# mburger-stsci/nexoclom

Measured on AMD Instinct MI355X. Metric: particle*steps/s, higher is better.
Workload: dtype f64

## Files before the change

### nexoclom_amd/csrc/nxc_api.hip

```cpp
#include <hip/hip_runtime.h>
#include <dlfcn.h>
#include <rccl/rccl.h>

#include <algorithm>
#include <atomic>
#include <cmath>
#include <cstddef>
#include <cstdio>
#include <cstdlib>
#include <cstring>
#include <ctime>
#include <limits>
#include <mutex>
#include <new>
#include <string>
#include <utility>
#include <vector>

#include "../../include/nexoclom_hip.h"
#include "nxc_camera_check.hpp"
#include "nxc_cube_check.hpp"
#include "nxc_desc_check.hpp"
#include "nxc_devbuf.hpp"
#include "nxc_image_block.hpp"
// ... 66 lines not shown
Rccl g_rccl;

int rccl_load()
{
    if (g_rccl.ok) return NXC_OK;
    const char *names[] = {"librccl.so.1", "librccl.so", "/opt/rocm/lib/librccl.so.1"};
    for (const char *nm : names) {
        g_rccl.lib = dlopen(nm, RTLD_NOW | RTLD_GLOBAL);
        if (g_rccl.lib) break;
    }
    if (!g_rccl.lib) return fail(NXC_ERR_RCCL, std::string("dlopen(librccl): ") + dlerror());
#define SYM(field, name)                                                                     \
    g_rccl.field = reinterpret_cast<decltype(g_rccl.field)>(dlsym(g_rccl.lib, name));        \
    if (!g_rccl.field) return fail(NXC_ERR_RCCL, std::string("dlsym ") + name + " failed");
    SYM(GetUniqueId, "ncclGetUniqueId")
    SYM(CommInitRank, "ncclCommInitRank")
    SYM(AllReduce, "ncclAllReduce")
    SYM(CommDestroy, "ncclCommDestroy")
    SYM(CommAbort, "ncclCommAbort")
    SYM(CommGetAsyncError, "ncclCommGetAsyncError")
    SYM(GetErrorString, "ncclGetErrorString")
#undef SYM
    g_rccl.ok = true;
    return NXC_OK;
}

#define NCCLCHK(expr)                                                                        \
    do {                                                                                     \
        ncclResult_t r_ = (expr);                                                            \
        if (r_ != ncclSuccess)                                                               \
            return fail(NXC_ERR_RCCL, std::string(#expr) + ": " + g_rccl.GetErrorString(r_)); \
    } while (0)

struct PackedLut {
    LutDesc desc{};
    std::vector<unsigned char> bytes;
};
struct LosLutCache {
    int64_t n = 0;
    std::vector<double> v, g;
    PackedLut lut;
};

int lut_cell_host(double x, double xbase, double inv_w, int ncell)
{
    const double s = (x - xbase) * inv_w;
    long long c;
    if (!(s >= 0.0)) c = 0;
    else if (s >= 2147483647.0) c = 2147483647ll;
    else c = (long long)s;
    return (int)std::min<long long>(c, ncell + 1);
}

unsigned long long ordered_key(double v)
{
    unsigned long long b;
    std::memcpy(&b, &v, sizeof b);
    return (b >> 63) ? ~b : (b | 0x8000000000000000ull);
}
double from_ordered_key(unsigned long long k)
{
    const unsigned long long b = (k >> 63) ? (k & 0x7fffffffffffffffull) : ~k;
    double v;
    std::memcpy(&v, &b, sizeof v);
    return v;
}

int pack_lut(const double *xp, const double *fp, int64_t n, PackedLut &out, const char *what,
             int cells_per_node = 4)
{
    if (n < 2 || n > 65000 || !xp || !fp)
        return fail(NXC_ERR_ARG, std::string(what) + ": table needs 2..65000 points");
    for (int64_t j = 0; j + 1 < n; j++)
        if (!(xp[j + 1] > xp[j]))
            return fail(NXC_ERR_ARG, std::string(what) + ": abscissae must be strictly ascending");
    for (int64_t j = 0; j < n; j++)
        if (!std::isfinite(xp[j]) || !std::isfinite(fp[j]))
            return fail(NXC_ERR_ARG, std::string(what) + ": table values must be finite");
    int ncell = 64;
    while (ncell < cells_per_node * n && ncell < 16384) ncell <<= 1;
    const int64_t rows = n + 2;
    const size_t cell_bytes = ((size_t)(ncell + 2) * sizeof(unsigned short) + 31) & ~size_t(31);
    out.bytes.assign((size_t)rows * 32 + cell_bytes, 0);
    double *rec = reinterpret_cast<double *>(out.bytes.data());
    double *fs = rec + 2 * rows;
    rec[0] = -std::numeric_limits<double>::max(); rec[1] = xp[0];
    fs[0] = fp[0]; fs[1] = 0.0;
    for (int64_t j = 0; j < n; j++) {
        const bool last = j + 1 == n;
        rec[2 * (j + 1)] = xp[j];
        rec[2 * (j + 1) + 1] = last ? HUGE_VAL : xp[j + 1];
        fs[2 * (j + 1)] = fp[j];
        fs[2 * (j + 1) + 1] = last ? 0.0 : (fp[j + 1] - fp[j]) / (xp[j + 1] - xp[j]);
        if (!std::isfinite(fs[2 * (j + 1) + 1]))
            return fail(NXC_ERR_ARG, std::string(what) + ": table slopes must be finite");
    }
    rec[2 * (n + 1)] = HUGE_VAL; rec[2 * (n + 1) + 1] = HUGE_VAL;
    fs[2 * (n + 1)] = fp[n - 1]; fs[2 * (n + 1) + 1] = 0.0;
    const double x0 = xp[0], xl = xp[n - 1];
    const double inv_w = (double)ncell / (xl - x0);
    const double xbase = x0 - (xl - x0) / (double)ncell;
    if (!std::isfinite(inv_w) || !std::isfinite(xbase) || !(xbase < x0))
        return fail(NXC_ERR_ARG, std::string(what) + ": abscissa range cannot be indexed");
    unsigned short *cell = reinterpret_cast<unsigned short *>(rec + 4 * rows);
    cell[0] = 0;
    const unsigned long long k_lo = ordered_key(-std::numeric_limits<double>::max());
    const unsigned long long k_hi = ordered_key(std::numeric_limits<double>::max());
    for (int c = 1; c <= ncell + 1; c++) {
        if (lut_cell_host(from_ordered_key(k_hi), xbase, inv_w, ncell) < c)
            return fail(NXC_ERR_ARG, std::string(what) + ": cell index is not onto");
        unsigned long long lo = k_lo, hi = k_hi;
        while (hi - lo > 1) {
            const unsigned long long mid = lo + (hi - lo) / 2;
            if (lut_cell_host(from_ordered_key(mid), xbase, inv_w, ncell) >= c) hi = mid;
            else lo = mid;
        }
        const double first = from_ordered_key(hi);
        const int64_t j = std::upper_bound(xp, xp + n, first) - xp;
        cell[c] = (unsigned short)j;
    }
    out.desc.rec = 0;
    out.desc.fs = 16 * (int)rows;
    out.desc.cell = 32 * (int)rows;
    out.desc.top = ncell + 1;
    out.desc.last = (int)n + 1;
    out.desc.xbase = xbase;
    out.desc.inv_w = inv_w;
    return NXC_OK;
}

int pack_lines(int n_lines, const double *const *v, const double *const *g, const int64_t *n, PackedLut *out)
{
    for (int l = 0; l < n_lines; l++) {
        int rc = pack_lut(v[l], g[l], n[l], out[l], "g-value table");
        if (rc) return rc;
    }
    return NXC_OK;
}

double sqrt_threshold(double e)
{
    if (!(e > 0) || !std::isfinite(e)) return e;
    double x = e * e;
    if (!std::isfinite(x)) return HUGE_VAL;
    while (std::sqrt(x) > e) x = std::nextafter(x, 0.0);
    while (std::sqrt(std::nextafter(x, HUGE_VAL)) <= e) x = std::nextafter(x, HUGE_VAL);
    return x;
}

StepW make_stepw(double h)
{
    StepW w{};
    w.h = h;
    for (int n = 0; n < 6; n++)
        for (int i = 0; i <= n; i++) w.w[n * (n + 1) / 2 + i] = h * Tableau::A[n + 1][i];
    return w;
}

void flush_all_pools();
struct HipAlloc {
    static inline thread_local hipError_t last = hipSuccess;
// ... 3787 lines not shown
```

### nexoclom_amd/csrc/nxc_device.hpp

```cpp
#pragma once
#include <hip/hip_runtime.h>
#include <stdint.h>
#include "nxc_math.hpp"
#include "nxc_fused_variant.hpp"

struct LutDesc {
    int rec, fs, cell;
    int top;
    int last;
    int pad_;
    double xbase;
    double inv_w;
};
typedef LutDesc LutView;

extern __shared__ __align__(32) unsigned char nxc_lds[];

#define NXC_LDS_AS __attribute__((address_space(3)))
#define NXC_GLOBAL_AS __attribute__((address_space(1)))
typedef double nxc_v2d __attribute__((ext_vector_type(2)));

NXC_DEV double lds_f64(int byte_off)
{
    return *(const NXC_LDS_AS double *)(unsigned)byte_off;
}
NXC_DEV int lds_u16(int byte_off)
{
    return *(const NXC_LDS_AS unsigned short *)(unsigned)byte_off;
}

NXC_DEV double2 lds_f64x2(int byte_off)
{
    const nxc_v2d v = *(const NXC_LDS_AS nxc_v2d *)(unsigned)byte_off;
    return make_double2(v.x, v.y);
}

NXC_DEV const LutView &lut_view(const LutDesc &d) { return d; }

NXC_DEV int lut_cell(const LutView &t, double x)
{
    const double s = (x - t.xbase) * t.inv_w;
    unsigned c;
    asm("v_cvt_u32_f64 %0, %1" : "=v"(c) : "v"(s));
    const unsigned top = (unsigned)t.top;
    return (int)(c > top ? top : c);
}

struct LutProbe {
    double x;
    int r;
    double2 a0, a1, b0, b1;
};

NXC_DEV void lut_probe_cell(const LutView &t, double x, LutProbe &p)
{
    p.x = x;
    p.r = lds_u16(t.cell + 2 * lut_cell(t, x));
}

NXC_DEV void lut_probe_rows(const LutView &t, LutProbe &p)
{
    const int ra = t.rec + 16 * p.r, rb = t.fs + 16 * p.r;
    p.a0 = lds_f64x2(ra); p.a1 = lds_f64x2(ra + 16);
    p.b0 = lds_f64x2(rb); p.b1 = lds_f64x2(rb + 16);
}

NXC_DEV LutProbe lut_probe(const LutView &t, double x)
{
    LutProbe p;
    lut_probe_cell(t, x, p);
    lut_probe_rows(t, p);
    return p;
}

NXC_DEV double lut_finish(const LutView &t, const LutProbe &p)
{
    const double x = p.x;
    const bool in0 = x < p.a0.y, in1 = x < p.a1.y;
    double xp = in0 ? p.a0.x : p.a1.x;
    double fp = in0 ? p.b0.x : p.b1.x;
    double sl = in0 ? p.b0.y : p.b1.y;
    if (__builtin_expect(!(in0 || in1), 0)) {
        int r = p.r + 1;
        while (r < t.last && x >= lds_f64(t.rec + 16 * r + 8)) ++r;
        const double2 aw = lds_f64x2(t.rec + 16 * r), bw = lds_f64x2(t.fs + 16 * r);
        xp = aw.x; fp = bw.x; sl = bw.y;
    }
    return sl * (x - xp) + fp;
}

NXC_DEV double lut_interp(const LutView &t, double x) { return lut_finish(t, lut_probe(t, x)); }

enum : int { LOSS_NONE = 0, LOSS_LIFETIME = 1, LOSS_PHOTO = 2 };

struct ForceK {
    double GM, vrplanet, photo, inv_lifetime;
    int grav, rad, loss, pad_;
    LutDesc tab;
};

NXC_DEV bool sunlit(double x, double y, double z)
{
    double s = x * x + z * z;
    return (s > 0x1.0000000000001p+0) || (y < 0.0);
}

template <bool FULL>
NXC_DEV void state_eval(const ForceK &F, const LutView &T, double x, double y, double z, double vy,
                        double &ax, double &ay, double &az, double &ion)
{
    const bool lit = sunlit(x, y, z);
    constexpr bool OVERLAP = FULL;
    LutProbe probe{};
    if (FULL || F.rad) lut_probe_cell(T, vy + F.vrplanet, probe);
    double gx = 0.0, gy = 0.0, gz = 0.0;
    if (FULL || F.grav) {
        const double s2 = (x * x + y * y) + z * z;
        const double nx = F.GM * x, ny = F.GM * y, nz = F.GM * z;
// ... 85 lines not shown
}

struct Tableau {
    static constexpr double A[7][7] = {
        {0, 0, 0, 0, 0, 0, 0},
        {0.2, 0, 0, 0, 0, 0, 0},
        {3. / 40., 9. / 40., 0, 0, 0, 0, 0},
        {44. / 45., -56. / 15., 32. / 9., 0, 0, 0, 0},
        {19372. / 6561., -25360. / 2187., 64448. / 6561., -212. / 729., 0, 0, 0},
        {9017. / 3168., -355. / 33., 46732. / 5247., 49. / 176., -5103. / 18656., 0, 0},
        {35. / 384., 0., 500. / 1113., 125. / 192., -2187. / 6784., 11. / 84., 0.}};
    static constexpr double B5[7] = {35. / 384., 0., 500. / 1113., 125. / 192., -2187. / 6784.,
                                     11. / 84., 0.};
    static constexpr double B4[7] = {5179. / 57600., 0., 7571. / 16695., 393. / 640.,
                                     -92097. / 339200., 187. / 2100., 1. / 40.};
};

struct StepW {
    double h;
    double w[21];
};

NXC_DEV double nxc_tab_fma(double w, double k, double acc)
{
#ifdef NXC_TABLEAU_TWO_ROUNDINGS
    return acc + w * k;
#else
    return __builtin_fma(w, k, acc);
#endif
}

template <bool DELTA, bool UNIFORM_H, bool FULL = false, bool NBODY = false>
NXC_DEV void rk5_step(const ForceK &F, const LutView &T, double (&s)[8], double h,
                      const StepW &W, double (&d)[8], const BodyK *Bd = nullptr,
                      const double *__restrict__ mp = nullptr)
{
    if (UNIFORM_H) h = W.h;
    double kv[6][3], ka[6][3], kl[6];
    const double x0 = s[1], y0 = s[2], z0 = s[3], vx0 = s[4], vy0 = s[5], vz0 = s[6];
    const double lf0 = nxc_log(s[7]);
    double px = x0, py = y0, pz = z0, vx = vx0, vy = vy0, vz = vz0, lf = lf0;
#pragma unroll
    for (int n = 0; n < 6; n++) {
        kv[n][0] = vx; kv[n][1] = vy; kv[n][2] = vz;
        state_eval<FULL>(F, T, px, py, pz, vy, ka[n][0], ka[n][1], ka[n][2], kl[n]);
        if (NBODY)
            bodies_eval(*Bd, mp, n, px, py, pz, vx, vy, vz, ka[n][0], ka[n][1], ka[n][2], kl[n]);
        double nx, ny, nz, nvx, nvy, nvz, nlf;
        {
            const double w = UNIFORM_H ? W.w[n * (n + 1) / 2] : h * Tableau::A[n + 1][0];
            nx = w * kv[0][0]; ny = w * kv[0][1]; nz = w * kv[0][2];
            nvx = w * ka[0][0]; nvy = w * ka[0][1]; nvz = w * ka[0][2];
            nlf = -(w * kl[0]);
        }
#pragma unroll
        for (int i = 1; i <= n; i++) {
            if (Tableau::A[n + 1][i] == 0.0) continue;
            const double w = UNIFORM_H ? W.w[n * (n + 1) / 2 + i] : h * Tableau::A[n + 1][i];
            nx = nxc_tab_fma(w, kv[i][0], nx);
            ny = nxc_tab_fma(w, kv[i][1], ny);
            nz = nxc_tab_fma(w, kv[i][2], nz);
            nvx = nxc_tab_fma(w, ka[i][0], nvx);
            nvy = nxc_tab_fma(w, ka[i][1], nvy);
            nvz = nxc_tab_fma(w, ka[i][2], nvz);
            nlf = nxc_tab_fma(-w, kl[i], nlf);
        }
        px = nx + x0; py = ny + y0; pz = nz + z0;
        vx = nvx + vx0; vy = nvy + vy0; vz = nvz + vz0;
        lf = nlf + lf0;
    }
    if (DELTA) {
        double e[7] = {0, 0, 0, 0, 0, 0, 0};
#pragma unroll
        for (int i = 0; i < 6; i++) {
            const double bd = Tableau::B5[i] - Tableau::B4[i];
            e[0] = nxc_tab_fma(bd, kv[i][0], e[0]);
            e[1] = nxc_tab_fma(bd, kv[i][1], e[1]);
            e[2] = nxc_tab_fma(bd, kv[i][2], e[2]);
            e[3] = nxc_tab_fma(bd, ka[i][0], e[3]);
            e[4] = nxc_tab_fma(bd, ka[i][1], e[4]);
            e[5] = nxc_tab_fma(bd, ka[i][2], e[5]);
            e[6] = nxc_tab_fma(bd, kl[i], e[6]);
        }
        d[0] = 0.0;
#pragma unroll
        for (int c = 0; c < 7; c++) d[c + 1] = __builtin_fabs(h * e[c]);
    }
    s[0] = (-h) + s[0];
    s[1] = px; s[2] = py; s[3] = pz; s[4] = vx; s[5] = vy; s[6] = vz;
    s[7] = nxc_exp(lf);
}
// ... 305 lines not shown
    R.vrplanet = G.vrplanet;
    R.xedges = (int)G.xedges_off; R.zedges = (int)G.zedges_off;
    R.nx = G.nx; R.nz = G.nz;
    R.x_lo = lds_f64(R.xedges); R.x_hi = lds_f64(R.xedges + 8 * R.nx);
    R.z_lo = lds_f64(R.zedges); R.z_hi = lds_f64(R.zedges + 8 * R.nz);
    R.x_inv_step = G.x_inv_step; R.z_inv_step = G.z_inv_step;
    R.quantity = G.quantity; R.n_lines = G.n_lines; R.downcast = G.downcast_f32;
    R.x_is_x = wave_uniform(G.x_is_x);
#ifdef NXC_EXPERIMENT_KNOBS
    R.dbg = G.dbg;
#else
    R.dbg = 0;
#endif
    R.vrplanet = wave_uniform(R.vrplanet);
    R.x_lo = wave_uniform(R.x_lo); R.x_hi = wave_uniform(R.x_hi);
    R.z_lo = wave_uniform(R.z_lo); R.z_hi = wave_uniform(R.z_hi);
    R.x_inv_step = wave_uniform(R.x_inv_step); R.z_inv_step = wave_uniform(R.z_inv_step);
    R.xedges = wave_uniform(R.xedges); R.zedges = wave_uniform(R.zedges);
    R.nx = wave_uniform(R.nx); R.nz = wave_uniform(R.nz);
    R.quantity = wave_uniform(R.quantity); R.n_lines = wave_uniform(R.n_lines);
    R.downcast = wave_uniform(R.downcast);
#ifdef NXC_EXPERIMENT_KNOBS
    R.dbg = wave_uniform(R.dbg);
#endif
    return R;
}

NXC_DEV double nxc_div_const(double n, double d, double y)
{
    if (!((nxc_mid_range(n) || n == 0.0) && y == y)) return n / d;
    return nxc_div_seeded(n, d, y);
}

NXC_DEV int bin_index(double v, int edges, int n, double lo, double hi, double inv_step)
{
    if (!(v >= lo) || !(v <= hi)) return -1;
    int k = (int)((v - lo) * inv_step);
    k = k > n - 1 ? n - 1 : k;
    const double e0 = lds_f64(edges + 8 * k), e1 = lds_f64(edges + 8 * k + 8);
    if (__builtin_expect(!((v >= e0) && (v < e1)), 0)) {
        while (k > 0 && v < lds_f64(edges + 8 * k)) --k;
        while (k < n - 1 && v >= lds_f64(edges + 8 * (k + 1))) ++k;
    }
    return k;
}

NXC_DEV double f32_round_trip(double v) { return (double)(float)v; }

NXC_DEV int half_swap(int v, bool upper)
{
    const auto r = __builtin_amdgcn_permlane32_swap(v, v, false, false);
    return upper ? (int)r[0] : (int)r[1];
}

NXC_DEV void image_add_pairs(bool has, int pix, double w, double *__restrict__ acc2)
{
    if (__ballot(has) == 0) return;
    const bool upper = (threadIdx.x & 32) != 0;
    const int ppix = half_swap(has ? pix : -1, upper);
    const bool own = has && w != 0.0;
    const bool partner = ppix >= 0;
    {
        const bool act = upper ? partner : own;
        if (act)
            unsafeAtomicAdd(&acc2[2ll * (upper ? ppix : pix) + (upper ? 1 : 0)], upper ? 1.0 : w);
    }
    {
        const bool act = upper ? own : partner;
        if (act)
            unsafeAtomicAdd(&acc2[2ll * (upper ? pix : ppix) + (upper ? 0 : 1)], upper ? w : 1.0);
    }
}

NXC_DEV double half_swap_f64(double v, bool upper)
{
    return __hiloint2double(half_swap(__double2hiint(v), upper), half_swap(__double2loint(v), upper));
}

NXC_DEV void add_record_pairs(bool has, int rec, double a, double b, double *__restrict__ rec2)
{
    if (__ballot(has) == 0) return;
    const bool upper = (threadIdx.x & 32) != 0;
    const int prec = half_swap(has ? rec : -1, upper);
    const double pb = half_swap_f64(b, upper);
    const bool partner = prec >= 0;
    {
        const bool act = upper ? partner : has;
        if (act)
            unsafeAtomicAdd(&rec2[2ll * (upper ? prec : rec) + (upper ? 1 : 0)], upper ? pb : a);
    }
    {
        const bool act = upper ? has : partner;
        if (act)
            unsafeAtomicAdd(&rec2[2ll * (upper ? rec : prec) + (upper ? 0 : 1)], upper ? a : pb);
    }
}

NXC_DEV bool image_locate_core_xz(const ImageK &G, const ImageRegs &R, double x, double y, double z,
                                  double vy, double frac, double &radvel_out, double &fw_out,
                                  unsigned long long &nonfinite, int &ix_out, int &iz_out)
{
    const double radvel = vy + R.vrplanet;
    double xo, yo, zo;
    if (R.x_is_x) {
        xo = x;
        yo = G.M[4] * y + G.M[5] * z;
        zo = G.M[7] * y + G.M[8] * z;
    } else {
        xo = (G.M[0] * x + G.M[1] * y) + G.M[2] * z;
        yo = (G.M[3] * x + G.M[4] * y) + G.M[5] * z;
        zo = (G.M[6] * x + G.M[7] * y) + G.M[8] * z;
    }
    const int ix = bin_index(xo, R.xedges, R.nx, R.x_lo, R.x_hi, R.x_inv_step);
    const int iz = bin_index(zo, R.zedges, R.nz, R.z_lo, R.z_hi, R.z_inv_step);
    if (ix < 0 || iz < 0) {
        if (!(__builtin_fabs(frac) <= 1.7976931348623157e308) || radvel != radvel) nonfinite++;
        return false;
    }
    const double s_obs = xo * xo + zo * zo;
    const bool inview = (s_obs > 0x1.0000000000001p+0) || (yo < 0.0);
    frac = inview ? frac : frac * 0.0;
    if (R.quantity != 0)
        frac = sunlit(x, y, z) ? frac : frac * 0.0;
    radvel_out = radvel;
    fw_out = frac;
    ix_out = ix; iz_out = iz;
    return true;
}

NXC_DEV int image_locate_core(const ImageK &G, const ImageRegs &R, double x, double y, double z,
                              double vy, double frac, double &radvel_out, double &fw_out,
                              unsigned long long &nonfinite)
{
    int ix = 0, iz = 0;
    if (!image_locate_core_xz(G, R, x, y, z, vy, frac, radvel_out, fw_out, nonfinite, ix, iz))
        return -1;
    return ix * R.nz + iz;
}

NXC_DEV int image_locate(const ImageK &G, const ImageRegs &R, double x, double y, double z,
                         double vy, double frac, double &radvel_out, double &fw_out,
                         unsigned long long &nonfinite)
{
    if (R.downcast) {
        x = f32_round_trip(x); y = f32_round_trip(y); z = f32_round_trip(z);
        vy = f32_round_trip(vy); frac = f32_round_trip(frac);
    }
    return image_locate_core(G, R, x, y, z, vy, frac, radvel_out, fw_out, nonfinite);
}

NXC_DEV bool image_frame_test(const ImageK &G, const ImageRegs &R, double x, double y, double z,
                              double vy, double frac, float &xf, float &yf, float &zf,
                              unsigned long long &nonfinite)
{
    xf = (float)x; yf = (float)y; zf = (float)z;
    const double xd = xf, yd = yf, zd = zf;
    double xo, zo;
    if (R.x_is_x) {
        xo = xd;
        zo = G.M[7] * yd + G.M[8] * zd;
    } else {
        xo = (G.M[0] * xd + G.M[1] * yd) + G.M[2] * zd;
        zo = (G.M[6] * xd + G.M[7] * yd) + G.M[8] * zd;
    }
    const bool inside = (xo >= R.x_lo) && (xo <= R.x_hi) && (zo >= R.z_lo) && (zo <= R.z_hi);
    if (!inside && (!(__builtin_fabs(frac) < 0x1.ffffffp127) || vy != vy)) nonfinite++;
    return inside;
}
// ... 235 lines not shown
```

### nexoclom_amd/csrc/nxc_image_block.hpp

```cpp
#pragma once
#include <cstddef>
#include <cstdint>
#include <vector>

#include "../../include/nexoclom_hip.h"

template <class Lut>
Lut placed_lut(Lut d, size_t base)
{
    d.rec += (int)base; d.fs += (int)base; d.cell += (int)base;
    return d;
}

template <class Lut>
struct ImageBlock {
    int n_lines = 0;
    Lut line[NXC_MAX_LINES]{};
    size_t xedges = 0, zedges = 0, bytes = 0;
};

template <class Image, class Packed>
auto append_image_block(std::vector<unsigned char> &out, Image &G, int64_t nx, int64_t nz,
                        const double *xedges, const double *zedges, int n_lines, const Packed *luts)
    -> ImageBlock<decltype(luts->desc)>
{
    ImageBlock<decltype(luts->desc)> b;
    const size_t start = out.size();
    b.n_lines = n_lines;
    for (int l = 0; l < n_lines; l++) {
        b.line[l] = placed_lut(luts[l].desc, out.size() - start);
        out.insert(out.end(), luts[l].bytes.begin(), luts[l].bytes.end());
    }
    b.xedges = out.size() - start;
    const unsigned char *xe = reinterpret_cast<const unsigned char *>(xedges);
    out.insert(out.end(), xe, xe + (nx + 1) * sizeof(double));
    b.zedges = out.size() - start;
    const unsigned char *ze = reinterpret_cast<const unsigned char *>(zedges);
    out.insert(out.end(), ze, ze + (nz + 1) * sizeof(double));
    b.bytes = out.size() - start;
    G.nx = (int)nx;
    G.nz = (int)nz;
    G.n_lines = n_lines;
    G.x_lo = xedges[0];
// ... 14 lines not shown
```

### nexoclom_amd/csrc/nxc_kernels.hpp

```cpp
#pragma once
#include "nxc_device.hpp"
#include "nxc_fused_variant.hpp"
#include "nxc_source_limits.hpp"
#include "nxc_tile_plan.hpp"

struct DevCounters {
    unsigned long long particle_steps, samples, samples_binned, nonfinite, bad_step, neg_frac,
        unfinished, queue_head;
    unsigned long long wave_trips;
#ifdef NXC_STAMPS
    unsigned long long stamp[8];
#endif
};

#ifdef NXC_STAMPS
NXC_DEV unsigned long long nxc_stamp()
{
    unsigned long long t;
    __builtin_amdgcn_sched_barrier(0);
    asm volatile("s_memtime %0\n\ts_waitcnt lgkmcnt(0)" : "=s"(t) : : "memory");
    __builtin_amdgcn_sched_barrier(0);
    return t;
}
#define NXC_STAMP(k) do { const unsigned long long t_ = nxc_stamp(); seg[k] += t_ - t_prev; t_prev = t_; } while (0)
// ... 91 lines not shown
    int hi = __builtin_amdgcn_readfirstlane((int)(v >> 32));
    return ((long long)hi << 32) | (unsigned int)lo;
}

__global__ void __launch_bounds__(NXC_BLOCK)
k_state(ForceK F, const unsigned char *__restrict__ blob, int64_t stage_bytes, int64_t n,
        const double *__restrict__ x, const double *__restrict__ y, const double *__restrict__ z,
        const double *__restrict__ vy, double *__restrict__ ax, double *__restrict__ ay,
        double *__restrict__ az, double *__restrict__ ion)
{
    stage_tables(blob, stage_bytes);
    const LutView T = lut_view(F.tab);
    for (int64_t i = (int64_t)blockIdx.x * blockDim.x + threadIdx.x; i < n;
         i += (int64_t)gridDim.x * blockDim.x) {
        double a0, a1, a2, l;
        state_eval<false>(F, T, x[i], y[i], z[i], vy[i], a0, a1, a2, l);
        ax[i] = a0; ay[i] = a1; az[i] = a2; ion[i] = l;
    }
}

template <bool DELTA>
__global__ void __launch_bounds__(NXC_BLOCK)
k_rk5_step(ForceK F, const unsigned char *__restrict__ blob, int64_t stage_bytes, int64_t n,
           const double *__restrict__ in, const double *__restrict__ hstep,
           double *__restrict__ out, double *__restrict__ delta)
{
    stage_tables(blob, stage_bytes);
    const LutView T = lut_view(F.tab);
    for (int64_t i = (int64_t)blockIdx.x * blockDim.x + threadIdx.x; i < n;
         i += (int64_t)gridDim.x * blockDim.x) {
        double s[8], d[8];
#pragma unroll
        for (int c = 0; c < 8; c++) s[c] = in[c * n + i];
        rk5_step<DELTA, false>(F, T, s, hstep[i], StepW{}, d);
#pragma unroll
        for (int c = 0; c < 8; c++) out[c * n + i] = s[c];
        if (DELTA) {
#pragma unroll
            for (int c = 0; c < 8; c++) delta[c * n + i] = d[c];
        }
    }
}

constexpr int NXC_REC_DOUBLES = 10;
constexpr int NXC_REC_FLOATS = 10;
typedef float nxc_v4f __attribute__((ext_vector_type(4)));
typedef float nxc_v2f __attribute__((ext_vector_type(2)));
typedef float nxc_v4f_a8 __attribute__((ext_vector_type(4), aligned(8)));

template <int ROWS>
NXC_DEV void store_record(void *__restrict__ rec, long long row, const double (&s)[8],
                          double lossfrac, long long id)
{
    if (ROWS == 2) {
        float *p = static_cast<float *>(rec) + row * NXC_REC_FLOATS;
        nxc_v4f a, b;
        nxc_v2f c;
        a.x = (float)s[0]; a.y = (float)s[1]; a.z = (float)s[2]; a.w = (float)s[3];
        b.x = (float)s[4]; b.y = (float)s[5]; b.z = (float)s[6]; b.w = (float)s[7];
        c.x = (float)lossfrac; c.y = __int_as_float((int)id);
        *reinterpret_cast<nxc_v4f_a8 *>(p) = a;
        *reinterpret_cast<nxc_v4f_a8 *>(p + 4) = b;
        *reinterpret_cast<nxc_v2f *>(p + 8) = c;
    } else {
        nxc_v2d *p = reinterpret_cast<nxc_v2d *>(static_cast<double *>(rec) + row * NXC_REC_DOUBLES);
        nxc_v2d a, b, c, d, e;
        a.x = s[0]; a.y = s[1]; b.x = s[2]; b.y = s[3]; c.x = s[4]; c.y = s[5]; d.x = s[6]; d.y = s[7];
// ... 146 lines not shown
                        stage[10 * NXC_CHUNK + lane] = __longlong_as_double(o1 - o0);
                    }
                }
                if (lane == 0) pending = claim(L.head);
                __builtin_amdgcn_fence(__ATOMIC_ACQUIRE, "wavefront");
                __builtin_amdgcn_wave_barrier();
            }
            const int room = c_cnt - c_pos;
            const int take = room < (want - served) ? room : want - served;
            if (need && rank >= served && rank < served + take) {
                const int slot = c_pos + (rank - served);
                mine = __double_as_longlong(stage[8 * NXC_CHUNK + slot]);
#pragma unroll
                for (int c = 0; c < 8; c++) s[c] = stage[c * NXC_CHUNK + slot];
                if (ROWS) {
                    *row0 = __double_as_longlong(stage[9 * NXC_CHUNK + slot]);
                    *nrow = __double_as_longlong(stage[10 * NXC_CHUNK + slot]);
                }
            }
            c_pos += take;
            served += take;
        }
        return mine;
    }
};

template <int IMAGE>
NXC_DEV bool image_pop(ImageQueue &queue, int imgq_off, const ImageRegs &IR, int &p, double &rv,
                       double &fw, unsigned long long &nonfinite)
{
    if (IMAGE == 2) {
        double x = 0, y = 0, z = 0, vy = 0, frac = 0;
        const bool ok = queue.pop_sample(imgq_off, x, y, z, vy, frac);
        if (ok) p = image_locate_core(lds_header().G, IR, x, y, z, vy, frac, rv, fw, nonfinite);
        return ok && p >= 0;
    }
    return queue.pop(imgq_off, p, rv, fw);
}

template <int IMAGE, bool BOUNCE, bool FULL, bool NBODY = false, int ROWS = 0, bool STREAMED = false>
__global__ void __launch_bounds__(NXC_BLOCK_PERSIST)
k_const_fused(ForceK F, const unsigned char *__restrict__ blob,
              int64_t stage_bytes, int64_t n, const double *__restrict__ soa0,
              const unsigned *__restrict__ order, int64_t first_id, int64_t n_iter,
              double edge2, double *__restrict__ final_out,
              long long *__restrict__ steps_out, double *__restrict__ acc2,
              DevCounters *__restrict__ ctr, const double *__restrict__ moon_pos = nullptr,
              const long long *__restrict__ offsets = nullptr, void *__restrict__ rec = nullptr,
              const unsigned long long *__restrict__ avail = nullptr)
{
    static_assert(!(IMAGE && ROWS), "the rows pass has no image");
    static_assert(!(STREAMED && (ROWS || BOUNCE || NBODY)), "the streamed pass is the plain one");
    stage_tables_and_args(blob, stage_bytes, soa0, order, final_out, steps_out, &ctr->queue_head, n,
                          offsets, STREAMED ? avail : nullptr);
    const LutView T = lut_view(F.tab);
    ImageRegs IR{};
    if (IMAGE) IR = image_regs(lds_header().G);
    ImageQueue queue;
    unsigned my_steps = 0, my_samples = 0, my_binned = 0;
    unsigned long long my_nonfinite = 0;
    WaveQueue q;
    q.start();
    const bool want_out = __builtin_amdgcn_readfirstlane(
        (final_out != nullptr || steps_out != nullptr) ? 1 : 0) != 0;
    const int wave_off = (int)((stage_bytes + 31) & ~31ll) +
                         (threadIdx.x >> 6) * (ROWS ? NXC_WAVE_LDS_BYTES_ROWS : NXC_WAVE_LDS_BYTES);
    const int stage_off = wave_off, imgq_off = wave_off + NXC_WAVE_STAGE_BYTES;
    bool has = false, fresh = false;
    long long id = -1, row0 = 0, nrow = 0;
    double lossfrac = 0.0;
    unsigned my_overrun = 0, my_trips = 0;
    int k = 0, nbounce = 0;
    const int n_it = n_iter > 0x7fffffffll ? 0x7fffffff : (int)n_iter;
    double s[8], d[8];
#ifdef NXC_STAMPS
    unsigned long long seg[8] = {0, 0, 0, 0, 0, 0, 0, 0}, t_prev = nxc_stamp();
#endif
    for (;;) {
#ifdef NXC_REFILL_MIN
        const unsigned long long free_ = __ballot(!has);
        const bool serve = __popcll(free_) >= NXC_REFILL_MIN || free_ == ~0ull;
        const long long got = serve ? q.refill<ROWS != 0, STREAMED>(!has, stage_off, s, &row0, &nrow) : -1;
#else
        const long long got = q.refill<ROWS != 0, STREAMED>(!has, stage_off, s, &row0, &nrow);
#endif
        if (got >= 0) { id = got; k = 0; has = true; fresh = true; nbounce = 0; lossfrac = 0.0; }
        if (__ballot(has) == 0) break;
        my_trips++;
        NXC_STAMP(0);
        int p = -1;
        double rv = 0.0, fw = 0.0;
        bool inframe = false;
        float qx = 0.f, qy = 0.f, qz = 0.f;
        if (has) {
            const double before = s[7];
            if (!fresh) {
                if (NBODY) {
                    const BodyK *Bd = &lds_header().Bd;
                    const double *mp = moon_pos + (long long)k * (2 * Bd->n_moons);
                    rk5_step<false, true, FULL, true>(F, T, s, 0.0, lds_header().W, d, Bd, mp);
                    apply_fate<false, true>(s, edge2, 0ull, nbounce, my_nonfinite, Bd, mp);
                } else {
                    rk5_step<false, true, FULL>(F, T, s, 0.0, lds_header().W, d);
                    apply_fate<BOUNCE>(s, edge2, (unsigned long long)(first_id + id), nbounce, my_nonfinite);
                }
#ifdef NXC_PROBE_VMOV
                {
                    int junk;
#pragma unroll
                    for (int j = 0; j < NXC_PROBE_VMOV; j++) asm volatile("v_mov_b32 %0, 0x12345" : "=v"(junk));
                }
#endif
#ifdef NXC_PROBE_FMA
                {
                    double j0 = s[1], j1 = s[2], j2 = s[3], j3 = s[4];
#pragma unroll
                    for (int j = 0; j < NXC_PROBE_FMA / 4; j++) {
                        asm volatile("v_fma_f64 %0, %0, %0, %0" : "+v"(j0));
                        asm volatile("v_fma_f64 %0, %0, %0, %0" : "+v"(j1));
                        asm volatile("v_fma_f64 %0, %0, %0, %0" : "+v"(j2));
                        asm volatile("v_fma_f64 %0, %0, %0, %0" : "+v"(j3));
                    }
                }
#endif
                k++; my_steps++;
                if (ROWS) lossfrac = (lossfrac + before) - s[7];
            }
            NXC_STAMP(1);
            fresh = false;
            const bool live = s[7] > 0.0;
            if (ROWS && live) {
                if (k < nrow) store_record<ROWS>(rec, row0 + k, s, lossfrac, id);
                else my_overrun++;
            }
            if (IMAGE && live) {
                my_samples++;
// ... 228 lines not shown
        if (__ballot(has) == 0) {
            if (!FAIR || !keeper || settled) break;
            const int simd = hw_simd();
            bool open = false;
            if (lane < nw) {
                const unsigned c = M.ld(M.hdr(lane));
                open = c == NXC_VAR_PENDING || (c != 0u && M.hdr(lane)[1] == (unsigned)simd && M.hdr(lane)[2] == 0u);
            }
            if (__ballot(open) == 0) break;
            __builtin_amdgcn_s_sleep(8);
            continue;
        }
        my_trips++;
        if (FAIR && !settled && (my_trips & 3u) == 0) {
            const unsigned long long t = __builtin_amdgcn_s_memrealtime();
            const int pr = (int)(((t >> NXC_VAR_PRIO_SHIFT) + (unsigned long long)hw_slot()) % 3ull);
            if (pr != prio) {
                prio = pr;
                if (pr == 2) __builtin_amdgcn_s_setprio(2);
                else if (pr == 1) __builtin_amdgcn_s_setprio(1);
                else __builtin_amdgcn_s_setprio(0);
            }
        }
        if (has) {
            bool done = !(s[0] > resolution && s[7] > 0.0);
            if (!done && it >= max_steps) { my_unfinished++; done = true; }
            if (!done) {
                const double h = __builtin_fmin(s[0], hs);
                if (!(h > 0.0)) { my_bad++; done = true; }
                else {
                    double t[8], d[8];
#pragma unroll
                    for (int c = 0; c < 8; c++) t[c] = s[c];
                    rk5_step<true, false, FULL>(F, T, t, h, StepW{}, d);
                    my_steps++; it++;
                    const double fscale = resf + __builtin_fabs(t[7]) * resf;
                    double e = d[0];
                    bool finite = true;
#pragma unroll
                    for (int c = 1; c <= 7; c++) {
                        const double scale = c <= 3 ? resx + __builtin_fabs(t[c]) * resx
                                           : c <= 6 ? resv + __builtin_fabs(t[c]) * resv : fscale;
                        const double q = nxc_div(d[c], scale);
                        finite = finite && (__builtin_fabs(q) <= 1.7976931348623157e308);
                        e = __builtin_fmax(e, q);
                    }
                    if (!finite) e = __builtin_nan("");
                    if (!(__builtin_fabs(e) <= 1.7976931348623157e308)) { my_nonfinite++; done = true; }
                    else {
                        if (t[7] < 0.0 && e < 1.0) my_neg++;
                        if ((t[7] - s[7] > fscale) && (e > 1.0)) e = 1.1;
                        double hold = h;
                        if (e < 1e-7) { e = 1.0; hold = h * 10; }
                        if (e < 1.0) {
                            { int nb_ = 0; apply_fate<false>(t, outeredge, 0ull, nb_, my_nonfinite); }
#pragma unroll
                            for (int c = 0; c < 8; c++) s[c] = t[c];
                        } else {
                            const double hn = 0.95 * hold * nxc_pow_m025(e);
                            if (!(__builtin_fabs(hn) <= 1.7976931348623157e308)) { my_bad++; done = true; }
                            else hs = __builtin_fmax(hn, 0.1 * hold);
                        }
                    }
                }
            }
            if (done) {
#pragma unroll
// ... 2046 lines not shown
```

Before: 33.84 billion.

## Fold LUT cell index into FMA and read RK weights from LDS

Precomputes c0 = -xbase*inv_w so the LUT cell lookup becomes a single FMA, and stores the fs-row offset relative to rec so the descriptor keeps one fewer base register. The RK5 step now loads its uniform weights and h straight from LDS at an offset instead of taking a StepW struct by value, with asm barriers to steer register and scalar/vector placement. Image binning in the in-frame sample path drops its redundant range checks through a template flag. Together these aim to cut VGPR pressure and ALU work per step, at the cost of extra LDS loads and small rounding differences in cell boundaries, which the host-side packer is updated to match.

```diff
diff --git a/nexoclom_amd/csrc/nxc_api.hip b/nexoclom_amd/csrc/nxc_api.hip
--- a/nexoclom_amd/csrc/nxc_api.hip
+++ b/nexoclom_amd/csrc/nxc_api.hip
@@ -122,101 +122,17 @@
             return fail(NXC_ERR_RCCL, std::string(#expr) + ": " + g_rccl.GetErrorString(r_)); \
     } while (0)
 
-struct PackedLut {
-    LutDesc desc{};
-    std::vector<unsigned char> bytes;
-};
 struct LosLutCache {
     int64_t n = 0;
     std::vector<double> v, g;
     PackedLut lut;
 };
 
-int lut_cell_host(double x, double xbase, double inv_w, int ncell)
-{
-    const double s = (x - xbase) * inv_w;
-    long long c;
-    if (!(s >= 0.0)) c = 0;
-    else if (s >= 2147483647.0) c = 2147483647ll;
-    else c = (long long)s;
-    return (int)std::min<long long>(c, ncell + 1);
-}
-
-unsigned long long ordered_key(double v)
-{
-    unsigned long long b;
-    std::memcpy(&b, &v, sizeof b);
-    return (b >> 63) ? ~b : (b | 0x8000000000000000ull);
-}
-double from_ordered_key(unsigned long long k)
-{
-    const unsigned long long b = (k >> 63) ? (k & 0x7fffffffffffffffull) : ~k;
-    double v;
-    std::memcpy(&v, &b, sizeof v);
-    return v;
-}
-
 int pack_lut(const double *xp, const double *fp, int64_t n, PackedLut &out, const char *what,
              int cells_per_node = 4)
 {
-    if (n < 2 || n > 65000 || !xp || !fp)
-        return fail(NXC_ERR_ARG, std::string(what) + ": table needs 2..65000 points");
-    for (int64_t j = 0; j + 1 < n; j++)
-        if (!(xp[j + 1] > xp[j]))
-            return fail(NXC_ERR_ARG, std::string(what) + ": abscissae must be strictly ascending");
-    for (int64_t j = 0; j < n; j++)
-        if (!std::isfinite(xp[j]) || !std::isfinite(fp[j]))
-            return fail(NXC_ERR_ARG, std::string(what) + ": table values must be finite");
-    int ncell = 64;
-    while (ncell < cells_per_node * n && ncell < 16384) ncell <<= 1;
-    const int64_t rows = n + 2;
-    const size_t cell_bytes = ((size_t)(ncell + 2) * sizeof(unsigned short) + 31) & ~size_t(31);
-    out.bytes.assign((size_t)rows * 32 + cell_bytes, 0);
-    double *rec = reinterpret_cast<double *>(out.bytes.data());
-    double *fs = rec + 2 * rows;
-    rec[0] = -std::numeric_limits<double>::max(); rec[1] = xp[0];
-    fs[0] = fp[0]; fs[1] = 0.0;
-    for (int64_t j = 0; j < n; j++) {
-        const bool last = j + 1 == n;
-        rec[2 * (j + 1)] = xp[j];
-        rec[2 * (j + 1) + 1] = last ? HUGE_VAL : xp[j + 1];
-        fs[2 * (j + 1)] = fp[j];
-        fs[2 * (j + 1) + 1] = last ? 0.0 : (fp[j + 1] - fp[j]) / (xp[j + 1] - xp[j]);
-        if (!std::isfinite(fs[2 * (j + 1) + 1]))
-            return fail(NXC_ERR_ARG, std::string(what) + ": table slopes must be finite");
-    }
-    rec[2 * (n + 1)] = HUGE_VAL; rec[2 * (n + 1) + 1] = HUGE_VAL;
-    fs[2 * (n + 1)] = fp[n - 1]; fs[2 * (n + 1) + 1] = 0.0;
-    const double x0 = xp[0], xl = xp[n - 1];
-    const double inv_w = (double)ncell / (xl - x0);
-    const double xbase = x0 - (xl - x0) / (double)ncell;
-    if (!std::isfinite(inv_w) || !std::isfinite(xbase) || !(xbase < x0))
-        return fail(NXC_ERR_ARG, std::string(what) + ": abscissa range cannot be indexed");
-    unsigned short *cell = reinterpret_cast<unsigned short *>(rec + 4 * rows);
-    cell[0] = 0;
-    const unsigned long long k_lo = ordered_key(-std::numeric_limits<double>::max());
-    const unsigned long long k_hi = ordered_key(std::numeric_limits<double>::max());
-    for (int c = 1; c <= ncell + 1; c++) {
-        if (lut_cell_host(from_ordered_key(k_hi), xbase, inv_w, ncell) < c)
-            return fail(NXC_ERR_ARG, std::string(what) + ": cell index is not onto");
-        unsigned long long lo = k_lo, hi = k_hi;
-        while (hi - lo > 1) {
-            const unsigned long long mid = lo + (hi - lo) / 2;
-            if (lut_cell_host(from_ordered_key(mid), xbase, inv_w, ncell) >= c) hi = mid;
-            else lo = mid;
-        }
-        const double first = from_ordered_key(hi);
-        const int64_t j = std::upper_bound(xp, xp + n, first) - xp;
-        cell[c] = (unsigned short)j;
-    }
-    out.desc.rec = 0;
-    out.desc.fs = 16 * (int)rows;
-    out.desc.cell = 32 * (int)rows;
-    out.desc.top = ncell + 1;
-    out.desc.last = (int)n + 1;
-    out.desc.xbase = xbase;
-    out.desc.inv_w = inv_w;
-    return NXC_OK;
+    const std::string why = pack_lut_rows(xp, fp, n, out, what, cells_per_node);
+    return why.empty() ? NXC_OK : fail(NXC_ERR_ARG, why);
 }
 
 int pack_lines(int n_lines, const double *const *v, const double *const *g, const int64_t *n, PackedLut *out)
diff --git a/nexoclom_amd/csrc/nxc_device.hpp b/nexoclom_amd/csrc/nxc_device.hpp
--- a/nexoclom_amd/csrc/nxc_device.hpp
+++ b/nexoclom_amd/csrc/nxc_device.hpp
@@ -3,15 +3,8 @@
 #include <stdint.h>
 #include "nxc_math.hpp"
 #include "nxc_fused_variant.hpp"
-
-struct LutDesc {
-    int rec, fs, cell;
-    int top;
-    int last;
-    int pad_;
-    double xbase;
-    double inv_w;
-};
+#include "nxc_lut_pack.hpp"
+
 typedef LutDesc LutView;
 
 extern __shared__ __align__(32) unsigned char nxc_lds[];
@@ -39,7 +32,7 @@
 
 NXC_DEV int lut_cell(const LutView &t, double x)
 {
-    const double s = (x - t.xbase) * t.inv_w;
+    const double s = __builtin_fma(x, t.inv_w, t.c0);
     unsigned c;
     asm("v_cvt_u32_f64 %0, %1" : "=v"(c) : "v"(s));
     const unsigned top = (unsigned)t.top;
@@ -60,7 +53,7 @@
 
 NXC_DEV void lut_probe_rows(const LutView &t, LutProbe &p)
 {
-    const int ra = t.rec + 16 * p.r, rb = t.fs + 16 * p.r;
+    const int ra = t.rec + 16 * p.r, rb = ra + t.to_fs;
     p.a0 = lds_f64x2(ra); p.a1 = lds_f64x2(ra + 16);
     p.b0 = lds_f64x2(rb); p.b1 = lds_f64x2(rb + 16);
 }
@@ -82,8 +75,9 @@
     double sl = in0 ? p.b0.y : p.b1.y;
     if (__builtin_expect(!(in0 || in1), 0)) {
         int r = p.r + 1;
+        asm volatile("" : "+v"(r));
         while (r < t.last && x >= lds_f64(t.rec + 16 * r + 8)) ++r;
-        const double2 aw = lds_f64x2(t.rec + 16 * r), bw = lds_f64x2(t.fs + 16 * r);
+        const double2 aw = lds_f64x2(t.rec + 16 * r), bw = lds_f64x2(t.rec + 16 * r + t.to_fs);
         xp = aw.x; fp = bw.x; sl = bw.y;
     }
     return sl * (x - xp) + fp;
@@ -235,10 +229,15 @@
 
 template <bool DELTA, bool UNIFORM_H, bool FULL = false, bool NBODY = false>
 NXC_DEV void rk5_step(const ForceK &F, const LutView &T, double (&s)[8], double h,
-                      const StepW &W, double (&d)[8], const BodyK *Bd = nullptr,
+                      int w_at, double (&d)[8], const BodyK *Bd = nullptr,
                       const double *__restrict__ mp = nullptr)
 {
-    if (UNIFORM_H) h = W.h;
+    int zero = 0;
+    if (UNIFORM_H) asm volatile("" : "+v"(zero));
+    const int w0 = zero + w_at + (int)offsetof(StepW, w);
+    if (UNIFORM_H) h = lds_f64(zero + w_at + (int)offsetof(StepW, h));
+    LutView Tv = T;
+    if (FULL) asm volatile("" : "+v"(Tv.c0));
     double kv[6][3], ka[6][3], kl[6];
     const double x0 = s[1], y0 = s[2], z0 = s[3], vx0 = s[4], vy0 = s[5], vz0 = s[6];
     const double lf0 = nxc_log(s[7]);
@@ -246,12 +245,12 @@
 #pragma unroll
     for (int n = 0; n < 6; n++) {
         kv[n][0] = vx; kv[n][1] = vy; kv[n][2] = vz;
-        state_eval<FULL>(F, T, px, py, pz, vy, ka[n][0], ka[n][1], ka[n][2], kl[n]);
+        state_eval<FULL>(F, Tv, px, py, pz, vy, ka[n][0], ka[n][1], ka[n][2], kl[n]);
         if (NBODY)
             bodies_eval(*Bd, mp, n, px, py, pz, vx, vy, vz, ka[n][0], ka[n][1], ka[n][2], kl[n]);
         double nx, ny, nz, nvx, nvy, nvz, nlf;
         {
-            const double w = UNIFORM_H ? W.w[n * (n + 1) / 2] : h * Tableau::A[n + 1][0];
+            const double w = UNIFORM_H ? lds_f64(w0 + 8 * (n * (n + 1) / 2)) : h * Tableau::A[n + 1][0];
             nx = w * kv[0][0]; ny = w * kv[0][1]; nz = w * kv[0][2];
             nvx = w * ka[0][0]; nvy = w * ka[0][1]; nvz = w * ka[0][2];
             nlf = -(w * kl[0]);
@@ -259,7 +258,7 @@
 #pragma unroll
         for (int i = 1; i <= n; i++) {
             if (Tableau::A[n + 1][i] == 0.0) continue;
-            const double w = UNIFORM_H ? W.w[n * (n + 1) / 2 + i] : h * Tableau::A[n + 1][i];
+            const double w = UNIFORM_H ? lds_f64(w0 + 8 * (n * (n + 1) / 2 + i)) : h * Tableau::A[n + 1][i];
             nx = nxc_tab_fma(w, kv[i][0], nx);
             ny = nxc_tab_fma(w, kv[i][1], ny);
             nz = nxc_tab_fma(w, kv[i][2], nz);
@@ -631,9 +630,10 @@
     return nxc_div_seeded(n, d, y);
 }
 
+template <bool INSIDE = false>
 NXC_DEV int bin_index(double v, int edges, int n, double lo, double hi, double inv_step)
 {
-    if (!(v >= lo) || !(v <= hi)) return -1;
+    if (!INSIDE && (!(v >= lo) || !(v <= hi))) return -1;
     int k = (int)((v - lo) * inv_step);
     k = k > n - 1 ? n - 1 : k;
     const double e0 = lds_f64(edges + 8 * k), e1 = lds_f64(edges + 8 * k + 8);
@@ -695,6 +695,7 @@
     }
 }
 
+template <bool INFRAME = false>
 NXC_DEV bool image_locate_core_xz(const ImageK &G, const ImageRegs &R, double x, double y, double z,
                                   double vy, double frac, double &radvel_out, double &fw_out,
                                   unsigned long long &nonfinite, int &ix_out, int &iz_out)
@@ -710,9 +711,9 @@
         yo = (G.M[3] * x + G.M[4] * y) + G.M[5] * z;
         zo = (G.M[6] * x + G.M[7] * y) + G.M[8] * z;
     }
-    const int ix = bin_index(xo, R.xedges, R.nx, R.x_lo, R.x_hi, R.x_inv_step);
-    const int iz = bin_index(zo, R.zedges, R.nz, R.z_lo, R.z_hi, R.z_inv_step);
-    if (ix < 0 || iz < 0) {
+    const int ix = bin_index<INFRAME>(xo, R.xedges, R.nx, R.x_lo, R.x_hi, R.x_inv_step);
+    const int iz = bin_index<INFRAME>(zo, R.zedges, R.nz, R.z_lo, R.z_hi, R.z_inv_step);
+    if (!INFRAME && (ix < 0 || iz < 0)) {
         if (!(__builtin_fabs(frac) <= 1.7976931348623157e308) || radvel != radvel) nonfinite++;
         return false;
     }
@@ -727,12 +728,13 @@
     return true;
 }
 
+template <bool INFRAME = false>
 NXC_DEV int image_locate_core(const ImageK &G, const ImageRegs &R, double x, double y, double z,
                               double vy, double frac, double &radvel_out, double &fw_out,
                               unsigned long long &nonfinite)
 {
     int ix = 0, iz = 0;
-    if (!image_locate_core_xz(G, R, x, y, z, vy, frac, radvel_out, fw_out, nonfinite, ix, iz))
+    if (!image_locate_core_xz<INFRAME>(G, R, x, y, z, vy, frac, radvel_out, fw_out, nonfinite, ix, iz))
         return -1;
     return ix * R.nz + iz;
 }
diff --git a/nexoclom_amd/csrc/nxc_image_block.hpp b/nexoclom_amd/csrc/nxc_image_block.hpp
--- a/nexoclom_amd/csrc/nxc_image_block.hpp
+++ b/nexoclom_amd/csrc/nxc_image_block.hpp
@@ -6,9 +6,15 @@
 #include "../../include/nexoclom_hip.h"
 
 template <class Lut>
+auto shift_second_rows(Lut &d, int base, int) -> decltype((void)d.fs) { d.fs += base; }
+template <class Lut>
+void shift_second_rows(Lut &, int, long) {}
+
+template <class Lut>
 Lut placed_lut(Lut d, size_t base)
 {
-    d.rec += (int)base; d.fs += (int)base; d.cell += (int)base;
+    d.rec += (int)base; d.cell += (int)base;
+    shift_second_rows(d, (int)base, 0);
     return d;
 }
 
diff --git a/nexoclom_amd/csrc/nxc_kernels.hpp b/nexoclom_amd/csrc/nxc_kernels.hpp
--- a/nexoclom_amd/csrc/nxc_kernels.hpp
+++ b/nexoclom_amd/csrc/nxc_kernels.hpp
@@ -147,7 +147,7 @@
         double s[8], d[8];
 #pragma unroll
         for (int c = 0; c < 8; c++) s[c] = in[c * n + i];
-        rk5_step<DELTA, false>(F, T, s, hstep[i], StepW{}, d);
+        rk5_step<DELTA, false>(F, T, s, hstep[i], 0, d);
 #pragma unroll
         for (int c = 0; c < 8; c++) out[c * n + i] = s[c];
         if (DELTA) {
@@ -360,7 +360,7 @@
     if (IMAGE == 2) {
         double x = 0, y = 0, z = 0, vy = 0, frac = 0;
         const bool ok = queue.pop_sample(imgq_off, x, y, z, vy, frac);
-        if (ok) p = image_locate_core(lds_header().G, IR, x, y, z, vy, frac, rv, fw, nonfinite);
+        if (ok) p = image_locate_core<true>(lds_header().G, IR, x, y, z, vy, frac, rv, fw, nonfinite);
         return ok && p >= 0;
     }
     return queue.pop(imgq_off, p, rv, fw);
@@ -426,10 +426,10 @@
                 if (NBODY) {
                     const BodyK *Bd = &lds_header().Bd;
                     const double *mp = moon_pos + (long long)k * (2 * Bd->n_moons);
-                    rk5_step<false, true, FULL, true>(F, T, s, 0.0, lds_header().W, d, Bd, mp);
+                    rk5_step<false, true, FULL, true>(F, T, s, 0.0, (int)offsetof(LdsHeader, W), d, Bd, mp);
                     apply_fate<false, true>(s, edge2, 0ull, nbounce, my_nonfinite, Bd, mp);
                 } else {
-                    rk5_step<false, true, FULL>(F, T, s, 0.0, lds_header().W, d);
+                    rk5_step<false, true, FULL>(F, T, s, 0.0, (int)offsetof(LdsHeader, W), d);
                     apply_fate<BOUNCE>(s, edge2, (unsigned long long)(first_id + id), nbounce, my_nonfinite);
                 }
 #ifdef NXC_PROBE_VMOV
@@ -724,7 +724,7 @@
                     double t[8], d[8];
 #pragma unroll
                     for (int c = 0; c < 8; c++) t[c] = s[c];
-                    rk5_step<true, false, FULL>(F, T, t, h, StepW{}, d);
+                    rk5_step<true, false, FULL>(F, T, t, h, 0, d);
                     my_steps++; it++;
                     const double fscale = resf + __builtin_fabs(t[7]) * resf;
                     double e = d[0];
diff --git a/nexoclom_amd/csrc/nxc_lut_pack.hpp b/nexoclom_amd/csrc/nxc_lut_pack.hpp
--- /dev/null
+++ b/nexoclom_amd/csrc/nxc_lut_pack.hpp
@@ -0,0 +1,116 @@
+#pragma once
+
+#include <algorithm>
+#include <cmath>
+#include <cstdint>
+#include <cstring>
+#include <limits>
+#include <string>
+#include <vector>
+
+struct LutDesc {
+    int rec, cell;
+    int to_fs;
+    int top;
+    int last;
+    int pad_;
+    double c0;
+    double inv_w;
+};
+
+struct PackedLut {
+    LutDesc desc{};
+    std::vector<unsigned char> bytes;
+};
+
+inline int lut_cell_host(double x, double c0, double inv_w, int ncell)
+{
+    const double s = std::fma(x, inv_w, c0);
+    long long c;
+    if (!(s >= 0.0)) c = 0;
+    else if (s >= 2147483647.0) c = 2147483647ll;
+    else c = (long long)s;
+    return (int)std::min<long long>(c, ncell + 1);
+}
+
+inline unsigned long long ordered_key(double v)
+{
+    unsigned long long b;
+    std::memcpy(&b, &v, sizeof b);
+    return (b >> 63) ? ~b : (b | 0x8000000000000000ull);
+}
+inline double from_ordered_key(unsigned long long k)
+{
+    const unsigned long long b = (k >> 63) ? (k & 0x7fffffffffffffffull) : ~k;
+    double v;
+    std::memcpy(&v, &b, sizeof v);
+    return v;
+}
+
+inline double lut_cell_first(int c, double c0, double inv_w, int ncell)
+{
+    unsigned long long lo = ordered_key(-std::numeric_limits<double>::max());
+    unsigned long long hi = ordered_key(std::numeric_limits<double>::max());
+    while (hi - lo > 1) {
+        const unsigned long long mid = lo + (hi - lo) / 2;
+        if (lut_cell_host(from_ordered_key(mid), c0, inv_w, ncell) >= c) hi = mid;
+        else lo = mid;
+    }
+    return from_ordered_key(hi);
+}
+
+inline std::string pack_lut_rows(const double *xp, const double *fp, int64_t n, PackedLut &out,
+                                 const char *what, int cells_per_node = 4)
+{
+    if (n < 2 || n > 65000 || !xp || !fp)
+        return std::string(what) + ": table needs 2..65000 points";
+    for (int64_t j = 0; j + 1 < n; j++)
+        if (!(xp[j + 1] > xp[j]))
+            return std::string(what) + ": abscissae must be strictly ascending";
+    for (int64_t j = 0; j < n; j++)
+        if (!std::isfinite(xp[j]) || !std::isfinite(fp[j]))
+            return std::string(what) + ": table values must be finite";
+    int ncell = 64;
+    while (ncell < cells_per_node * n && ncell < 16384) ncell <<= 1;
+    const int64_t rows = n + 2;
+    const size_t cell_bytes = ((size_t)(ncell + 2) * sizeof(unsigned short) + 31) & ~size_t(31);
+    out.bytes.assign((size_t)rows * 32 + cell_bytes, 0);
+    double *rec = reinterpret_cast<double *>(out.bytes.data());
+    double *fs = rec + 2 * rows;
+    rec[0] = -std::numeric_limits<double>::max(); rec[1] = xp[0];
+    fs[0] = fp[0]; fs[1] = 0.0;
+    for (int64_t j = 0; j < n; j++) {
+        const bool last = j + 1 == n;
+        rec[2 * (j + 1)] = xp[j];
+        rec[2 * (j + 1) + 1] = last ? HUGE_VAL : xp[j + 1];
+        fs[2 * (j + 1)] = fp[j];
+        fs[2 * (j + 1) + 1] = last ? 0.0 : (fp[j + 1] - fp[j]) / (xp[j + 1] - xp[j]);
+        if (!std::isfinite(fs[2 * (j + 1) + 1]))
+            return std::string(what) + ": table slopes must be finite";
+    }
+    rec[2 * (n + 1)] = HUGE_VAL; rec[2 * (n + 1) + 1] = HUGE_VAL;
+    fs[2 * (n + 1)] = fp[n - 1]; fs[2 * (n + 1) + 1] = 0.0;
+    const double x0 = xp[0], xl = xp[n - 1];
+    const double inv_w = (double)ncell / (xl - x0);
+    const double xbase = x0 - (xl - x0) / (double)ncell;
+    const double c0 = -(xbase * inv_w);
+    if (!std::isfinite(inv_w) || !std::isfinite(xbase) || !(xbase < x0) || !std::isfinite(c0))
+        return std::string(what) + ": abscissa range cannot be indexed";
+    unsigned short *cell = reinterpret_cast<unsigned short *>(rec + 4 * rows);
+    cell[0] = 0;
+    if (lut_cell_host(std::numeric_limits<double>::max(), c0, inv_w, ncell) < ncell + 1)
+        return std::string(what) + ": cell index is not onto";
+    for (int c = 1; c <= ncell + 1; c++) {
+        const double first = lut_cell_first(c, c0, inv_w, ncell);
+        const int64_t j = std::upper_bound(xp, xp + n, first) - xp;
+        cell[c] = (unsigned short)j;
+    }
+    out.desc.rec = 0;
+    out.desc.cell = 32 * (int)rows;
+    out.desc.to_fs = 16 * (int)rows;
+    out.desc.top = ncell + 1;
+    out.desc.last = (int)n + 1;
+    out.desc.c0 = c0;
+    out.desc.inv_w = inv_w;
+    return std::string();
+}
```

New measurement: 34.19 billion, median of 5. 1.01x the previous value.
